# notu97/GS-SLAM-Analytica_Jacobian

Measured on AMD Instinct MI355X. Metric: Gaussian-pixel interactions/sec (fwd+Jacobian), 640x480, higher is better.
Workload: dtype f32; 1 GPU; cfg2: 50000 Gaussians (SH degree 3, 16 coeffs), 640x480; one step = one mapping window of 8 keyframes with distinct cameras: forward splat + analytical-Jacobian backward (dL/dmu, dL/dSigma->conic, per-Gaussian grads summed over the window, one dL/dtau per keyframe)

## Files before the change

gs-slam-analytica_jacobian_amd/csrc/preprocess.hip:

```cpp
#include "gsaj_common.h"
#include "wave_reduce.h"

__constant__ float kSH_C0 = 0.28209479177387814f;
__constant__ float kSH_C1 = 0.4886025119029199f;
__constant__ float kSH_C2[5] = {1.0925484305920792f, -1.0925484305920792f, 0.31539156525252005f, -1.0925484305920792f,
                                0.5462742152960396f};
__constant__ float kSH_C3[7] = {-0.5900435899266435f, 2.890611442640554f, -0.4570457994644658f, 0.3731763325901154f,
                                -0.4570457994644658f, 1.445305721320277f, -0.5900435899266435f};

__device__ __forceinline__ float3 ld3(const float *p, size_t i) { return make_float3(p[3 * i], p[3 * i + 1], p[3 * i + 2]); }

__device__ __forceinline__ void cov3d_from_scale_rot(float3 sc, float mod, float4 q, float *c6) {
  const float r = q.x, x = q.y, y = q.z, z = q.w;
  float R[3][3] = {{1.f - 2.f * (y * y + z * z), 2.f * (x * y - r * z), 2.f * (x * z + r * y)},
                   {2.f * (x * y + r * z), 1.f - 2.f * (x * x + z * z), 2.f * (y * z - r * x)},
                   {2.f * (x * z - r * y), 2.f * (y * z + r * x), 1.f - 2.f * (x * x + y * y)}};
  const float s[3] = {mod * sc.x, mod * sc.y, mod * sc.z};
  float A[3][3];
#pragma unroll
  for (int i = 0; i < 3; i++)
#pragma unroll
    for (int j = 0; j < 3; j++) A[i][j] = s[i] * R[j][i];
  float S[3][3];
#pragma unroll
  for (int a = 0; a < 3; a++)
#pragma unroll
    for (int b = a; b < 3; b++) S[a][b] = A[0][a] * A[0][b] + A[1][a] * A[1][b] + A[2][a] * A[2][b];
  c6[0] = S[0][0]; c6[1] = S[0][1]; c6[2] = S[0][2]; c6[3] = S[1][1]; c6[4] = S[1][2]; c6[5] = S[2][2];
}

__device__ __forceinline__ float3 cov2d_forward(float3 mean, float fx, float fy, float tanx, float tany, const float *c6,
                                                const float *vm) {
  float3 t = xform4x3(vm, mean);
  const float limx = 1.3f * tanx, limy = 1.3f * tany;
  const float txtz = t.x / t.z, tytz = t.y / t.z;
  t.x = fminf(limx, fmaxf(-limx, txtz)) * t.z;
  t.y = fminf(limy, fmaxf(-limy, tytz)) * t.z;
  const float J00 = fx / t.z, J02 = -(fx * t.x) / (t.z * t.z);
  const float J11 = fy / t.z, J12 = -(fy * t.y) / (t.z * t.z);
  float M[2][3];
#pragma unroll
  for (int k = 0; k < 3; k++) {
    M[0][k] = vm[4 * k + 0] * J00 + vm[4 * k + 1] * 0.0f + vm[4 * k + 2] * J02;
    M[1][k] = vm[4 * k + 0] * 0.0f + vm[4 * k + 1] * J11 + vm[4 * k + 2] * J12;
  }
  const float V[3][3] = {{c6[0], c6[1], c6[2]}, {c6[1], c6[3], c6[4]}, {c6[2], c6[4], c6[5]}};
  float X[2][3];
#pragma unroll
  for (int r = 0; r < 2; r++)
#pragma unroll
    for (int c = 0; c < 3; c++) X[r][c] = M[r][0] * V[c][0] + M[r][1] * V[c][1] + M[r][2] * V[c][2];
  float3 cov;
  cov.x = (X[0][0] * M[0][0] + X[0][1] * M[0][1] + X[0][2] * M[0][2]) + 0.3f;
  cov.y = X[1][0] * M[0][0] + X[1][1] * M[0][1] + X[1][2] * M[0][2];
  cov.z = (X[1][0] * M[1][0] + X[1][1] * M[1][1] + X[1][2] * M[1][2]) + 0.3f;
  return cov;
}

__device__ __forceinline__ float3 sh_to_rgb(int deg, float3 pos, float3 campos, const float *sh, uint8_t *clamped) {
  float3 d = make_float3(pos.x - campos.x, pos.y - campos.y, pos.z - campos.z);
  const float len = sqrtf(d.x * d.x + d.y * d.y + d.z * d.z);
  const float x = d.x / len, y = d.y / len, z = d.z / len;
  float out[3];
#pragma unroll
  for (int ch = 0; ch < 3; ch++) {
#define SHC(k) sh[(k) * 3 + ch]
    float res = kSH_C0 * SHC(0);
    if (deg > 0) {
      res = res - kSH_C1 * y * SHC(1) + kSH_C1 * z * SHC(2) - kSH_C1 * x * SHC(3);
      if (deg > 1) {
        const float xx = x * x, yy = y * y, zz = z * z, xy = x * y, yz = y * z, xz = x * z;
        res = res + kSH_C2[0] * xy * SHC(4) + kSH_C2[1] * yz * SHC(5) + kSH_C2[2] * (2.0f * zz - xx - yy) * SHC(6) +
              kSH_C2[3] * xz * SHC(7) + kSH_C2[4] * (xx - yy) * SHC(8);
        if (deg > 2) {
          res = res + kSH_C3[0] * y * (3.0f * xx - yy) * SHC(9) + kSH_C3[1] * xy * z * SHC(10) +
                kSH_C3[2] * y * (4.0f * zz - xx - yy) * SHC(11) + kSH_C3[3] * z * (2.0f * zz - 3.0f * xx - 3.0f * yy) * SHC(12) +
                kSH_C3[4] * x * (4.0f * zz - xx - yy) * SHC(13) + kSH_C3[5] * z * (xx - yy) * SHC(14) +
                kSH_C3[6] * x * (xx - 3.0f * yy) * SHC(15);
        }
      }
    }
#undef SHC
    res += 0.5f;
    clamped[ch] = (res < 0.0f);
    out[ch] = res < 0.0f ? 0.0f : res;
  }
  return make_float3(out[0], out[1], out[2]);
}

GSAJ_TRACE_DEFINE(pre)

template <bool SH16, bool MULTI>
__global__ __launch_bounds__(PRE_BLOCK) void k_preprocess(FwdParams p, int *__restrict__ radii, int *__restrict__ n_touched,
                                                         GeomWS g, ImageWS im, ViewStrides vs) {
  __shared__ uint32_t scan[PRE_BLOCK / 64];
  extern __shared__ uint32_t hist[];
  {
    const size_t view = blockIdx.y;
    g = geom_view(g, view * vs.geom);
    im = image_view(im, view * vs.image);
    p.viewmatrix += 16 * view;
    p.projmatrix += 16 * view;
    if (p.campos) p.campos += 3 * view;
    radii += view * (size_t)p.P;
    n_touched += view * (size_t)p.P;
  }
  GSAJ_TRACE_BEGIN(pre)
#ifdef GSAJ_BLOCK_TRACE
  unsigned long long trp_[4] = {0, 0, 0, 0}, trp_t = wall_clock64();
#define TRP(i) { const unsigned long long n_ = wall_clock64(); trp_[i] += n_ - trp_t; trp_t = n_; }
#else
#define TRP(i)
#endif
  const int tid = threadIdx.x;
  const int tiles = p.grid_x * p.grid_y;
  const bool use_lds = tiles <= LDS_TILES_MAX;
  if (use_lds) {
    for (int t = tid; t < tiles; t += PRE_BLOCK) hist[t] = 0u;
    __syncthreads();
  }
  const int nblk_all = (p.P + PRE_BLOCK - 1) / PRE_BLOCK;
#pragma clang loop unroll(disable)
  for (int it = 0; it < (MULTI ? p.bpw : 1); it++) {
  const int blk = MULTI ? (int)blockIdx.x * p.bpw + it : (int)blockIdx.x;
  if (blk >= nblk_all) break;
  const int idx = blk * PRE_BLOCK + tid;
  uint32_t touched = 0;
  uint32_t rect_x = 0, rect_y = 0;
  float depth = 0.f;
  if (idx < p.P) {
    int my_radius_i = 0;
    uint32_t rect_pack = 0;
    float2 xy = make_float2(0.f, 0.f);
    float4 con_o = make_float4(0.f, 0.f, 0.f, 0.f);
    float3 rgb = make_float3(0.f, 0.f, 0.f);
    uint8_t cl[3] = {0, 0, 0};
    float c6s[6] = {0.f, 0.f, 0.f, 0.f, 0.f, 0.f};
    const float3 p_orig = ld3(p.means3D, idx);
    float3 sc_in = make_float3(0.f, 0.f, 0.f);
    float4 q_in = make_float4(1.f, 0.f, 0.f, 0.f);
    if (!p.cov3D_precomp) {
      sc_in = ld3(p.scales, idx);
      q_in = reinterpret_cast<const float4 *>(p.rotations)[idx];
    }
    const float opac_in = p.opacities[idx];
    constexpr bool sh_regs = SH16;
    float shv[SH16 ? 48 : 1];
    if (sh_regs) {
      const float4 *s4 = reinterpret_cast<const float4 *>(p.shs + (size_t)idx * 48);
#pragma unroll
      for (int k = 0; k < 12; k++) {
        const float4 t = s4[k];
        shv[4 * k] = t.x; shv[4 * k + 1] = t.y; shv[4 * k + 2] = t.z; shv[4 * k + 3] = t.w;
      }
    }
    const float3 p_view = xform4x3(p.viewmatrix, p_orig);
    if (p_view.z <= 0.2f) {
      if (p.prefiltered) atomicOr(&im.counters[1], ERR_PREFILTERED);
    } else {
      const float4 p_hom = xform4x4(p.projmatrix, p_orig);
      const float p_w = 1.0f / (p_hom.w + 0.0000001f);
      const float3 p_proj = make_float3(p_hom.x * p_w, p_hom.y * p_w, p_hom.z * p_w);
      float c6[6];
      if (p.cov3D_precomp) {
#pragma unroll
        for (int k = 0; k < 6; k++) c6[k] = p.cov3D_precomp[6 * (size_t)idx + k];
      } else {
        cov3d_from_scale_rot(sc_in, p.scale_modifier, q_in, c6s);
#pragma unroll
        for (int k = 0; k < 6; k++) c6[k] = c6s[k];
      }
      const float3 cov = cov2d_forward(p_orig, p.focal_x, p.focal_y, p.tanfovx, p.tanfovy, c6, p.viewmatrix);
      const float det = cov.x * cov.z - cov.y * cov.y;
      if (det != 0.0f) {
        const float det_inv = 1.f / det;
        const float3 conic = make_float3(cov.z * det_inv, -cov.y * det_inv, cov.x * det_inv);
        const float mid = 0.5f * (cov.x + cov.z);
        const float sq = sqrtf(fmaxf(0.1f, mid * mid - det));
        const float lambda1 = mid + sq, lambda2 = mid - sq;
        const float my_radius = ceilf(3.f * sqrtf(fmaxf(lambda1, lambda2)));
        const float2 pim = make_float2(ndc2pix(p_proj.x, p.W), ndc2pix(p_proj.y, p.H));
        int x0, y0, x1, y1;
        tile_rect(pim.x, pim.y, (int)my_radius, p.grid_x, p.grid_y, gsaj_tile_band(im.sticky), x0, y0, x1, y1);
        const int area = (x1 - x0) * (y1 - y0);
        if (area != 0) {
          if (!p.colors_precomp) {
            const float3 cam = make_float3(p.campos[0], p.campos[1], p.campos[2]);
            if constexpr (sh_regs) rgb = sh_to_rgb(p.D, p_orig, cam, shv, cl);
            else rgb = sh_to_rgb(p.D, p_orig, cam, p.shs + (size_t)idx * p.M * 3, cl);
          }
          rect_pack = (uint32_t)x0 | ((uint32_t)y0 << 10) | ((uint32_t)(x1 - x0) << 20);
          rect_x = (uint32_t)x0 | ((uint32_t)x1 << 16);
          rect_y = (uint32_t)y0 | ((uint32_t)y1 << 16);
          depth = p_view.z;
          my_radius_i = (int)my_radius;
          xy = pim;
          con_o = make_float4(conic.x, conic.y, conic.z, opac_in);
          touched = (uint32_t)area;
          for (int y = y0; y < y1; y++)
            for (int x = x0; x < x1; x++) {
              if (use_lds) atomicAdd(&hist[y * p.grid_x + x], 1u);
              else atomicAdd(&im.tile_count[y * p.grid_x + x], 1u);
            }
        }
      }
    }
    radii[idx] = my_radius_i;
    n_touched[idx] = 0;
    g.depths[idx] = depth;
    if (!p.cov3D_precomp && blockIdx.y == 0) {
#pragma unroll
      for (int k = 0; k < 6; k++) g.cov3D[6 * (size_t)idx + k] = c6s[k];
    }
    if (!p.colors_precomp) {
      g.clamped[3 * (size_t)idx] = cl[0]; g.clamped[3 * (size_t)idx + 1] = cl[1]; g.clamped[3 * (size_t)idx + 2] = cl[2];
    }
    g.tiles_touched[idx] = touched;
    if (p.colors_precomp) rgb = ld3(p.colors_precomp, idx);
    g.splat[3 * (size_t)idx + 0] = make_float4(xy.x, xy.y, __uint_as_float(rect_pack), 0.f);
    g.splat[3 * (size_t)idx + 1] = con_o;
    g.splat[3 * (size_t)idx + 2] = make_float4(rgb.x, rgb.y, rgb.z, depth);
  }
  TRP(0)
  uint32_t incl = touched;
  {
    const int lane = tid & 63;
#pragma unroll
    for (int o = 1; o < 64; o <<= 1) {
      const uint32_t v = (uint32_t)__shfl_up((int)incl, o);
      if (lane >= o) incl += v;
    }
    if (lane == 63) scan[tid >> 6] = incl;
  }
  __syncthreads();
  uint32_t block_total = 0;
#pragma unroll
  for (int w = 0; w < PRE_BLOCK / 64; w++) {
    const uint32_t v = scan[w];
    if (w < (tid >> 6)) incl += v;
    block_total += v;
  }
  if (idx < p.P) {
    const uint32_t first = incl - touched;
    g.point_offsets[idx] = incl;
    reinterpret_cast<float *>(g.splat)[12 * (size_t)idx + 3] = __uint_as_float(first);
    g.scat[idx] = make_uint2(rect_x, rect_y);
  }
  if (tid == 0) g.block_sums[blk] = block_total;
  __syncthreads();
  }
  if (use_lds)
    for (int t = tid; t < tiles; t += PRE_BLOCK) {
      const uint32_t c = hist[t];
      if (c) atomicAdd(&im.tile_count[t], c);
    }
  TRP(1)
  GSAJ_TRACE_END(pre)
#ifdef GSAJ_BLOCK_TRACE
  if ((threadIdx.x & 63) == 0) {
    unsigned long long *t = g_trace_pre + 4 * (blockIdx.x * (PRE_BLOCK / 64) + (threadIdx.x >> 6));
    t[2] = (trp_[0] << 32) | trp_[1];
    t[3] = 0;
  }
#endif
}

__device__ uint32_t tail_exclusive_scan(const uint32_t *in, uint32_t *out, int n, uint32_t *run_max) {
  __shared__ uint32_t wsum[PRE_BLOCK / 64];
  __shared__ uint32_t wmax[PRE_BLOCK / 64];
  const int tid = threadIdx.x, lane = tid & 63, wave = tid >> 6;
  const int per = (n + PRE_BLOCK - 1) / PRE_BLOCK;
  const int b0 = min(n, tid * per), b1 = min(n, b0 + per);
  uint32_t s = 0, mx = 0;
  for (int i = b0; i < b1; i++) {
    const uint32_t v = in[i];
    s += v;
    mx = max(mx, v);
  }
  uint32_t incl = s;
#pragma unroll
  for (int o = 1; o < 64; o <<= 1) {
    const uint32_t v = __shfl_up((int)incl, o);
    if (lane >= o) incl += v;
  }
#pragma unroll
  for (int o = 32; o > 0; o >>= 1) mx = max(mx, (uint32_t)__shfl_xor((int)mx, o));
  if (lane == 63) wsum[wave] = incl;
  if (lane == 0) wmax[wave] = mx;
  __syncthreads();
  uint32_t woff = 0, total = 0, m = 0;
#pragma unroll
  for (int w = 0; w < PRE_BLOCK / 64; w++) {
    const uint32_t v = wsum[w];
    if (w < wave) woff += v;
    total += v;
    m = max(m, wmax[w]);
  }
  if (run_max) *run_max = m;
  uint32_t run = woff + incl - s;
  for (int i = b0; i < b1; i++) {
    const uint32_t v = in[i];
    out[i] = run;
    run += v;
  }
  __syncthreads();
  return total;
}

__device__ uint32_t tile_scan_and_schedule(int tiles, ImageWS im, uint32_t *len, uint32_t *longest_out) {
  __shared__ uint32_t wsum[PRE_BLOCK / 64], wmax[PRE_BLOCK / 64], cls[64];
  const int tid = threadIdx.x, lane = tid & 63, wave = tid >> 6;
  for (int c = tid; 4 * c < tiles; c += PRE_BLOCK) {
    const uint4 v = *reinterpret_cast<const uint4 *>(im.tile_count + 4 * c);
    len[4 * c] = v.x;
    if (4 * c + 1 < tiles) len[4 * c + 1] = v.y;
    if (4 * c + 2 < tiles) len[4 * c + 2] = v.z;
    if (4 * c + 3 < tiles) len[4 * c + 3] = v.w;
  }
  if (tid < 64) cls[tid] = 0u;
  __syncthreads();
  const int per = (tiles + PRE_BLOCK - 1) / PRE_BLOCK;
  const int b0 = min(tiles, tid * per), b1 = min(tiles, b0 + per);
  uint32_t s = 0, mx = 0;
  for (int i = b0; i < b1; i++) {
    s += len[i];
    mx = max(mx, len[i]);
  }
  uint32_t incl = s;
#pragma unroll
  for (int o = 1; o < 64; o <<= 1) {
    const uint32_t v = __shfl_up((int)incl, o);
    if (lane >= o) incl += v;
  }
#pragma unroll
  for (int o = 32; o > 0; o >>= 1) mx = max(mx, (uint32_t)__shfl_xor((int)mx, o));
  if (lane == 63) wsum[wave] = incl;
  if (lane == 0) wmax[wave] = mx;
  __syncthreads();
  uint32_t woff = 0, total = 0, longest = 0;
#pragma unroll
  for (int w = 0; w < PRE_BLOCK / 64; w++) {
    const uint32_t v = wsum[w];
    if (w < wave) woff += v;
    total += v;
    longest = max(longest, wmax[w]);
  }
  uint32_t run = woff + incl - s;
  for (int i = b0; i < b1; i++) {
    im.tile_offset[i] = run;
    run += len[i];
  }
  const int shift = longest >= 64u ? (32 - __builtin_clz(longest)) - 6 : 0;
  for (int t = tid; t < tiles; t += PRE_BLOCK) atomicAdd(&cls[63u - min(63u, len[t] >> shift)], 1u);
  __syncthreads();
  if (tid < 64) {
    const uint32_t v = cls[tid];
    uint32_t in2 = v;
#pragma unroll
    for (int o = 1; o < 64; o <<= 1) {
      const uint32_t u = (uint32_t)__shfl_up((int)in2, o);
      if (tid >= o) in2 += u;
    }
    cls[tid] = in2 - v;
  }
  __syncthreads();
  for (int t = tid; t < tiles; t += PRE_BLOCK) im.tile_order[atomicAdd(&cls[63u - min(63u, len[t] >> shift)], 1u)] = (uint32_t)t;
  __syncthreads();
  *longest_out = longest;
  return total;
}

__global__ __launch_bounds__(PRE_BLOCK) void k_frame_scan(int nblk, int tiles, int capacity, GeomWS g, ImageWS im, ViewStrides vs) {
  extern __shared__ uint32_t lds_len[];
  g = geom_view(g, (size_t)blockIdx.y * vs.geom);
  im = image_view(im, (size_t)blockIdx.y * vs.image);
  uint32_t *block_sums = g.block_sums;
  const uint32_t R = tail_exclusive_scan(block_sums, block_sums, nblk, nullptr);
  uint32_t m = 0, R2;
  if (tiles <= LDS_TILES_MAX) {
    R2 = tile_scan_and_schedule(tiles, im, lds_len, &m);
  } else {
    R2 = tail_exclusive_scan(im.tile_count, im.tile_offset, tiles, &m);
    for (int t = threadIdx.x; t < tiles; t += PRE_BLOCK) im.tile_order[t] = (uint32_t)t;
  }
  if (threadIdx.x == 0) {
    im.tile_offset[tiles] = R2;
    im.counters[0] = R;
    im.counters[2] = m;
    uint32_t err = 0u;
    if (R2 != R) err |= ERR_INTERNAL;
    if (capacity > 0) {
      if (R > (uint32_t)capacity) err |= ERR_CAPACITY;
      if (err) {
        im.counters[4] = 1u;
        atomicAdd(&im.sticky[0], 1u);
      }
    }
    if (err) atomicOr(&im.counters[1], err);
  }
}

#ifndef SCAT_CLS
#define SCAT_CLS 8
#endif
#define SCAT_LDS_TILES 4096
#define SCAT_STAGE 4096
GSAJ_TRACE_DEFINE(scat)

__global__ __launch_bounds__(PRE_BLOCK) void k_scatter_instances(int P, int gx, int gy, int gpt, GeomWS g, ImageWS im,
                                                                 uint32_t *__restrict__ inst_id, ViewStrides vs) {
  extern __shared__ uint32_t lds[];
  __shared__ uint32_t stage_id[SCAT_STAGE];
  __shared__ uint16_t stage_lt[SCAT_STAGE];
  __shared__ uint32_t s_wave[PRE_BLOCK / 64], s_carry;
  {
    const size_t view = blockIdx.y;
    g = geom_view(g, view * vs.geom);
    im = image_view(im, view * vs.image);
    inst_id = gsaj_shift(inst_id, view * vs.bin);
  }
  if (im.counters[4]) return;
  GSAJ_TRACE_BEGIN(scat)
#ifdef GSAJ_BLOCK_TRACE
  unsigned long long trs_[4] = {0, 0, 0, 0}, trs_t = wall_clock64();
#define TRS(i) { const unsigned long long n_ = wall_clock64(); trs_[i] += n_ - trs_t; trs_t = n_; }
#else
#define TRS(i)
#endif
  const int tid = threadIdx.x;
  const int cls = (int)(blockIdx.x % SCAT_CLS), gb = (int)(blockIdx.x / SCAT_CLS);
  const int rows_c = (gy - cls + SCAT_CLS - 1) / SCAT_CLS;
  const int ltiles = rows_c > 0 ? rows_c * gx : 0;
  const bool use_lds = ((gy + SCAT_CLS - 1) / SCAT_CLS) * gx <= SCAT_LDS_TILES;
  uint32_t *cnt = lds, *fill = lds + ltiles, *lbase = lds + 2 * ltiles;
  if (use_lds) {
    for (int t = tid; t < 2 * ltiles; t += PRE_BLOCK) lds[t] = 0u;
    if (tid == 0) s_carry = 0u;
    __syncthreads();
  }
#define SCAT_FOR_EACH_TILE(BODY)                                                                     \
  for (int i0 = 0; i0 < gpt; i0 += 4) {                                                              \
    uint2 sc[4];                                                                                     \
    _Pragma("unroll") for (int j = 0; j < 4; j++) {                                                  \
      const int idx = (gb * gpt + i0 + j) * PRE_BLOCK + tid;                                         \
      sc[j] = (i0 + j < gpt && idx < P) ? g.scat[idx] : make_uint2(0u, 0u);                          \
    }                                                                                                \
    _Pragma("unroll") for (int j = 0; j < 4; j++) {                                                  \
      const int x0 = (int)(sc[j].x & 0xffffu), x1 = (int)(sc[j].x >> 16);                            \
      const int y0 = (int)(sc[j].y & 0xffffu), y1 = (int)(sc[j].y >> 16);                            \
      if (x1 > x0) {                                                                                 \
        const uint32_t id = (uint32_t)((gb * gpt + i0 + j) * PRE_BLOCK + tid);                       \
        (void)id;                                                                                    \
        const int ys = y0 + ((cls - y0) % SCAT_CLS + SCAT_CLS) % SCAT_CLS;                           \
        for (int y = ys; y < y1; y += SCAT_CLS)                                                      \
          for (int x = x0; x < x1; x++) {                                                            \
            const int lt = (y / SCAT_CLS) * gx + x;                            \
            const int t = y * gx + x;                                                      \
            (void)lt; (void)t;                                                                       \
            BODY                                                                                     \
          }                                                                                          \
      }                                                                                              \
    }                                                                                                \
  }
  if (!use_lds) {
    SCAT_FOR_EACH_TILE({ inst_id[im.tile_offset[t] + atomicAdd(&im.tile_cursor[t], 1u)] = id; })
    return;
  }
  TRS(0)
  SCAT_FOR_EACH_TILE({ atomicAdd(&cnt[lt], 1u); })
  __syncthreads();
  TRS(1)
  for (int l0 = 0; l0 < ltiles; l0 += PRE_BLOCK) {
    const int lt = l0 + tid, lane = tid & 63;
    uint32_t c = 0u, off = 0u, base = 0u;
    if (lt < ltiles) {
      const int j = lt / gx;
      const int t = (j * SCAT_CLS + cls) * gx + (lt - j * gx);
      c = cnt[lt];
      off = im.tile_offset[t];
      if (c) base = atomicAdd(&im.tile_cursor[t], c);
    }
    uint32_t incl = c;
#pragma unroll
    for (int o = 1; o < 64; o <<= 1) {
      const uint32_t v = (uint32_t)__shfl_up((int)incl, o);
      if (lane >= o) incl += v;
    }
    if (lane == 63) s_wave[tid >> 6] = incl;
    __syncthreads();
    uint32_t before = s_carry;
#pragma unroll
    for (int w = 0; w < PRE_BLOCK / 64; w++)
      if (w < (tid >> 6)) before += s_wave[w];
    if (lt < ltiles) {
      cnt[lt] = off + base;
      lbase[lt] = before + incl - c;
    }
    __syncthreads();
    if (tid == PRE_BLOCK - 1) s_carry = before + incl;
  }
  __syncthreads();
  const uint32_t total = s_carry;
  TRS(2)
  if (total <= SCAT_STAGE) {
    SCAT_FOR_EACH_TILE({
      const uint32_t k = atomicAdd(&fill[lt], 1u);
      stage_id[lbase[lt] + k] = id;
      stage_lt[lbase[lt] + k] = (uint16_t)lt;
    })
    __syncthreads();
    for (uint32_t i = tid; i < total; i += PRE_BLOCK) {
      const uint32_t lt = stage_lt[i];
      inst_id[cnt[lt] + (i - lbase[lt])] = stage_id[i];
    }
  } else {
    SCAT_FOR_EACH_TILE({ inst_id[cnt[lt] + atomicAdd(&fill[lt], 1u)] = id; })
  }
#undef SCAT_FOR_EACH_TILE
  TRS(3)
  GSAJ_TRACE_END(scat)
#ifdef GSAJ_BLOCK_TRACE
  if ((threadIdx.x & 63) == 0) {
    const unsigned tw_ = (blockIdx.y * gridDim.x + blockIdx.x) * (blockDim.x >> 6) + (threadIdx.x >> 6);
    if (tw_ < GSAJ_TRACE_MAX) {
      g_trace_scat[4 * tw_ + 2] = (trs_[0] << 32) | trs_[1];
      g_trace_scat[4 * tw_ + 3] = (trs_[2] << 32) | trs_[3];
    }
  }
#endif
}

__global__ __launch_bounds__(256) void k_pack_splat16(int P, GeomWS g, const uint32_t *__restrict__ counters, ViewStrides vs) {
  g = geom_view(g, (size_t)blockIdx.y * vs.geom);
  if (gsaj_shift(counters, (size_t)blockIdx.y * vs.image)[4]) return;
  const int idx = blockIdx.x * 256 + threadIdx.x;
  if (idx >= P) return;
  const float4 a = g.splat[3 * (size_t)idx + 0], bq = g.splat[3 * (size_t)idx + 1], c = g.splat[3 * (size_t)idx + 2];
  g.splat16[2 * (size_t)idx + 0] = make_float4(a.x, a.y, c.w, a.w);
  g.splat16[2 * (size_t)idx + 1] = make_float4(__uint_as_float(gsaj_pack_h2(bq.x, bq.y)), __uint_as_float(gsaj_pack_h2(bq.z, bq.w)),
                                              __uint_as_float(gsaj_pack_h2(c.x, c.y)), __uint_as_float(gsaj_pack_h2(c.z, 0.f)));
}

template <int J>
__device__ __forceinline__ uint32_t lane_xor(uint32_t x, int lane) {
  if (J == 32) {
    const gsaj_u32x2 r = __builtin_amdgcn_permlane32_swap(x, x, false, false);
    return lane < 32 ? r[1] : r[0];
  } else if (J == 16) {
    const gsaj_u32x2 r = __builtin_amdgcn_permlane16_swap(x, x, false, false);
    return (lane & 16) ? r[0] : r[1];
  } else if (J == 8) {
    return (uint32_t)__builtin_amdgcn_mov_dpp((int)x, 0x128, 0xF, 0xF, true);
  } else if (J == 4) {
    int t = __builtin_amdgcn_mov_dpp((int)x, 0x104, 0xF, 0x5, false);
    t = __builtin_amdgcn_update_dpp(t, (int)x, 0x114, 0xF, 0xA, false);
    return (uint32_t)t;
  } else if (J == 2) {
    return (uint32_t)__builtin_amdgcn_mov_dpp((int)x, 0x4E, 0xF, 0xF, true);
  } else {
    return (uint32_t)__builtin_amdgcn_mov_dpp((int)x, 0xB1, 0xF, 0xF, true);
  }
}
template <int MASK>
__device__ __forceinline__ uint32_t lane_mirror(uint32_t x, int lane) {
  if (MASK == 1) return (uint32_t)__builtin_amdgcn_mov_dpp((int)x, 0xB1, 0xF, 0xF, true);
  else if (MASK == 3) return (uint32_t)__builtin_amdgcn_mov_dpp((int)x, 0x1B, 0xF, 0xF, true);
  else if (MASK == 7) return (uint32_t)__builtin_amdgcn_mov_dpp((int)x, 0x141, 0xF, 0xF, true);
  else if (MASK == 15) return (uint32_t)__builtin_amdgcn_mov_dpp((int)x, 0x140, 0xF, 0xF, true);
  else if (MASK == 31) return lane_xor<16>(lane_mirror<15>(x, lane), lane);
  else return lane_xor<32>(lane_mirror<31>(x, lane), lane);
}
template <int MASK>
__device__ __forceinline__ uint64_t key_mirror(uint64_t k, int lane) {
  return ((uint64_t)lane_mirror<MASK>((uint32_t)(k >> 32), lane) << 32) | lane_mirror<MASK>((uint32_t)k, lane);
}

#define KEY_INF 0x7FEFFFFFFFFFFFFFull
__device__ __forceinline__ void key_minmax(uint64_t a, uint64_t b, uint64_t &lo, uint64_t &hi) {
  double l, h;
  asm("v_min_f64 %0, %2, %3\n\tv_max_f64 %1, %2, %3" : "=&v"(l), "=&v"(h) : "v"(__longlong_as_double((long long)a)), "v"(__longlong_as_double((long long)b)));
  lo = (uint64_t)__double_as_longlong(l);
  hi = (uint64_t)__double_as_longlong(h);
}
__device__ __forceinline__ uint64_t key_min(uint64_t a, uint64_t b) {
  double l;
  asm("v_min_f64 %0, %1, %2" : "=v"(l) : "v"(__longlong_as_double((long long)a)), "v"(__longlong_as_double((long long)b)));
  return (uint64_t)__double_as_longlong(l);
}
__device__ __forceinline__ uint64_t key_max(uint64_t a, uint64_t b) {
  double h;
  asm("v_max_f64 %0, %1, %2" : "=v"(h) : "v"(__longlong_as_double((long long)a)), "v"(__longlong_as_double((long long)b)));
  return (uint64_t)__double_as_longlong(h);
}
template <int J>
__device__ __forceinline__ constexpr uint64_t lower_lanes() {
  return J == 1 ? 0x5555555555555555ull : J == 2 ? 0x3333333333333333ull : J == 4 ? 0x0F0F0F0F0F0F0F0Full
       : J == 8 ? 0x00FF00FF00FF00FFull : J == 16 ? 0x0000FFFF0000FFFFull : 0x00000000FFFFFFFFull;
}
__device__ __forceinline__ void key_stage(uint64_t &A, uint64_t XA, uint64_t YA, uint64_t &B, uint64_t XB, uint64_t YB, uint64_t lower) {
  double a, b2;
  uint64_t save;
  asm volatile("s_mov_b64 %[sv], exec\n\t"
               "s_and_b64 exec, %[sv], %[lo]\n\t"
               "v_min_f64 %[a], %[xa], %[ya]\n\t"
               "v_min_f64 %[b], %[xb], %[yb]\n\t"
               "s_andn2_b64 exec, %[sv], %[lo]\n\t"
               "v_max_f64 %[a], %[xa], %[ya]\n\t"
               "v_max_f64 %[b], %[xb], %[yb]\n\t"
               "s_mov_b64 exec, %[sv]\n\t"
               "s_nop 4"
               : [a] "=&v"(a), [b] "=&v"(b2), [sv] "=&s"(save)
               : [xa] "v"(__longlong_as_double((long long)XA)), [ya] "v"(__longlong_as_double((long long)YA)),
                 [xb] "v"(__longlong_as_double((long long)XB)), [yb] "v"(__longlong_as_double((long long)YB)), [lo] "s"(lower)
               : "scc");
  A = (uint64_t)__double_as_longlong(a);
  B = (uint64_t)__double_as_longlong(b2);
}
template <int J>
__device__ __forceinline__ void key_both(uint64_t k, uint64_t &of_lower, uint64_t &of_upper) {
  const uint32_t hi = (uint32_t)(k >> 32), lo = (uint32_t)k;
  gsaj_u32x2 rh, rl;
  if (J == 32) {
    rh = __builtin_amdgcn_permlane32_swap(hi, hi, false, false);
    rl = __builtin_amdgcn_permlane32_swap(lo, lo, false, false);
    of_lower = ((uint64_t)rh[0] << 32) | rl[0];
    of_upper = ((uint64_t)rh[1] << 32) | rl[1];
  } else {
    rh = __builtin_amdgcn_permlane16_swap(hi, hi, false, false);
    rl = __builtin_amdgcn_permlane16_swap(lo, lo, false, false);
    of_lower = ((uint64_t)rh[0] << 32) | rl[0];
    of_upper = ((uint64_t)rh[1] << 32) | rl[1];
  }
}
template <int J>
__device__ __forceinline__ void sort_stage(uint64_t &A, uint64_t &B, int lane) {
  if constexpr (J >= 16) {
    uint64_t al, au, bl, bu;
    key_both<J>(A, al, au);
    key_both<J>(B, bl, bu);
    key_stage(A, al, au, B, bl, bu, lower_lanes<J>());
  } else {
    const uint64_t PA = ((uint64_t)lane_xor<J>((uint32_t)(A >> 32), lane) << 32) | lane_xor<J>((uint32_t)A, lane);
    const uint64_t PB = ((uint64_t)lane_xor<J>((uint32_t)(B >> 32), lane) << 32) | lane_xor<J>((uint32_t)B, lane);
    key_stage(A, A, PA, B, B, PB, lower_lanes<J>());
  }
}
template <int J>
__device__ __forceinline__ void merge_strides(uint64_t &A, uint64_t &B, int lane) {
  if constexpr (J == 64) {
    key_minmax(A, B, A, B);
  } else {
    sort_stage<J>(A, B, lane);
  }
  if constexpr (J > 1) merge_strides<J / 2>(A, B, lane);
}
template <int K>
__device__ __forceinline__ void local_merge(uint64_t &A, uint64_t &B, int lane) {
  if constexpr (K == 128) {
    const uint64_t PA = key_mirror<63>(B, lane), PB = key_mirror<63>(A, lane);
    A = key_min(A, PA);
    B = key_max(B, PB);
    merge_strides<32>(A, B, lane);
  } else {
    const uint64_t PA = key_mirror<K - 1>(A, lane), PB = key_mirror<K - 1>(B, lane);
    key_stage(A, A, PA, B, B, PB, lower_lanes<K / 2>());
    if constexpr (K >= 4) merge_strides<K / 4>(A, B, lane);
  }
}
template <int K>
__device__ __forceinline__ void local_merges(uint64_t &A, uint64_t &B, int lane, int m) {
  if (K > m) return;
  local_merge<K>(A, B, lane);
  if constexpr (K < 128) local_merges<2 * K>(A, B, lane, m);
}

template <int NT>
__device__ __forceinline__ void lds_bitonic_sort(uint64_t *keys, int n, int tid) {
  const int lane = tid & 63, wave = tid >> 6;
  const int nch = (n + 127) >> 7, nup = nch << 7;
  int m = 2;
  while (m < n) m <<= 1;
  for (int chunk = wave; chunk < nch; chunk += NT / 64) {
    const int ia = chunk * 128 + lane, ib = ia + 64;
    uint64_t A = keys[ia], B = keys[ib];
    local_merges<2>(A, B, lane, m);
    keys[ia] = A;
    keys[ib] = B;
  }
  __syncthreads();
  for (int k = 256, hs = 7; (k >> 1) < nup; k <<= 1, hs++) {
    const int half = k >> 1;
    for (int i = tid; i < (nup >> 1) + half; i += NT) {
      const int blk = i >> hs, off = i & (half - 1);
      const int l = (blk << (hs + 1)) + off, r = (blk << (hs + 1)) + k - 1 - off;
      if (r < nup) key_minmax(keys[l], keys[r], keys[l], keys[r]);
    }
    __syncthreads();
    for (int j = k >> 2; j >= 128; j >>= 1) {
      for (int i = tid; i < (nup >> 1); i += NT) {
        const int l = ((i & ~(j - 1)) << 1) | (i & (j - 1)), r = l + j;
        if (r < nup && ((l & ~(k - 1)) + half) < nup) key_minmax(keys[l], keys[r], keys[l], keys[r]);
      }
      __syncthreads();
    }
    for (int chunk = wave; chunk < nch; chunk += NT / 64) {
      if (((chunk * 128) & ~(k - 1)) + half >= nup) continue;
      const int ia = chunk * 128 + lane, ib = ia + 64;
      uint64_t A = keys[ia], B = keys[ib];
      merge_strides<64>(A, B, lane);
      keys[ia] = A;
      keys[ib] = B;
    }
    __syncthreads();
  }
}

template <int NT>
__device__ __forceinline__ void lds_bitonic_merge(uint64_t *keys, int T, int tid) {
  const int lane = tid & 63, wave = tid >> 6;
  for (int j = T >> 1; j >= 128; j >>= 1) {
    for (int i = tid; i < (T >> 1); i += NT) {
      const int l = ((i & ~(j - 1)) << 1) | (i & (j - 1)), r = l + j;
      key_minmax(keys[l], keys[r], keys[l], keys[r]);
    }
    __syncthreads();
  }
  for (int chunk = wave; chunk * 128 < T; chunk += NT / 64) {
    const int ia = chunk * 128 + lane, ib = ia + 64;
    uint64_t A = keys[ia], B = keys[ib];
    merge_strides<64>(A, B, lane);
    keys[ia] = A;
    keys[ib] = B;
  }
  __syncthreads();
}

template <int NT>
__device__ const uint64_t *sort_long_list(uint64_t *lds, int T, uint32_t *split_s, const uint32_t *ids, const float *__restrict__ depths,
                                          uint64_t *a, uint64_t *b, int n, int tid) {
  for (int c0 = 0; c0 < n; c0 += T) {
    const int len = min(T, n - c0);
    for (int i0 = tid; i0 < T; i0 += 4 * NT) {
      uint32_t id[4], dz[4];
#pragma unroll
      for (int u = 0; u < 4; u++) id[u] = ids[c0 + min(i0 + u * NT, len - 1)];
#pragma unroll
      for (int u = 0; u < 4; u++) dz[u] = __float_as_uint(depths[id[u]]);
#pragma unroll
      for (int u = 0; u < 4; u++) asm volatile("" : "+v"(dz[u]));
#pragma unroll
      for (int u = 0; u < 4; u++) {
        const int i = i0 + u * NT;
        if (i < T) lds[i] = i < len ? ((uint64_t)dz[u] << 32) | id[u] : KEY_INF;
      }
    }
    __syncthreads();
    lds_bitonic_sort<NT>(lds, T, tid);
    for (int i = tid; i < len; i += NT) b[c0 + i] = lds[i];
    __syncthreads();
  }
  uint64_t *src = b, *dst = a;
  for (long long width = T; width < (long long)n; width <<= 1) {
    asm volatile("s_waitcnt vmcnt(0)" ::: "memory");
    __syncthreads();
    for (long long p0 = 0; p0 < (long long)n; p0 += 2 * width) {
      const int la = (int)min(width, (long long)n - p0);
      const int lb = (int)max(0ll, min(width, (long long)n - p0 - width));
      const uint64_t *A = src + p0, *B = src + p0 + width;
      uint64_t *D = dst + p0;
      if (lb == 0) {
        for (int i = tid; i < la; i += NT) D[i] = A[i];
        continue;
      }
      const int tot = la + lb, nblk = (tot + T - 1) / T;
      for (int j0 = 0; j0 < nblk; j0 += PRE_BLOCK) {
        for (int t = tid; t <= PRE_BLOCK; t += NT) {
          const long long dl = (long long)(j0 + t) * T;
          const int d = (int)min(dl, (long long)tot);
          int lo = max(0, d - lb), hi = min(d, la);
          while (lo < hi) {
            const int mid = (lo + hi) >> 1;
            if (A[mid] <= B[d - 1 - mid]) lo = mid + 1;
            else hi = mid;
          }
          split_s[t] = (uint32_t)lo;
        }
        __syncthreads();
        for (int j = j0; j < min(nblk, j0 + PRE_BLOCK); j++) {
          const int a0 = (int)split_s[j - j0], a1 = (int)split_s[j - j0 + 1];
          const int d0 = j * T, d1 = min(tot, d0 + T);
          const int b0 = d0 - a0, cA = a1 - a0, cB = (d1 - a1) - b0;
          for (int i = tid; i < T; i += NT) lds[i] = i < cA ? A[a0 + i] : (i >= T - cB ? B[b0 + (T - 1 - i)] : KEY_INF);
          __syncthreads();
          lds_bitonic_merge<NT>(lds, T, tid);
          for (int i = tid; i < cA + cB; i += NT) D[d0 + i] = lds[i];
          __syncthreads();
        }
      }
    }
    uint64_t *t = src;
    src = dst;
    dst = t;
  }
  asm volatile("s_waitcnt vmcnt(0)" ::: "memory");
  __syncthreads();
  return src;
}

GSAJ_TRACE_DEFINE(sort)

#ifndef GSAJ_SORT_128_MAX
#define GSAJ_SORT_128_MAX 1024
#endif
template <int NT>
__global__ __launch_bounds__(NT) void k_tile_sort(ImageWS im, const float *__restrict__ depths, uint64_t *__restrict__ inst_key,
                                                   uint64_t *__restrict__ keys_b, uint32_t *point_list,
                                                   uint8_t *__restrict__ reached, int cap, int pass, int rec16, ViewStrides vs) {
  {
    const size_t view = blockIdx.y;
    im = image_view(im, view * vs.image);
    depths = gsaj_shift(depths, view * vs.geom);
    inst_key = gsaj_shift(inst_key, view * vs.bin);
    keys_b = gsaj_shift(keys_b, view * vs.bin);
    point_list = gsaj_shift(point_list, view * vs.bin);
    reached = gsaj_shift(reached, view * vs.bin);
  }
  extern __shared__ uint64_t keys[];
  if (im.counters[4]) return;
  GSAJ_TRACE_BEGIN(sort)
#ifdef GSAJ_BLOCK_TRACE
  unsigned long long tr_a = wall_clock64(), tr_b = 0, tr_c = 0;
#endif
  const int tid = threadIdx.x, tile = blockIdx.x;
  const uint32_t beg = im.tile_offset[tile * TILE_REP], end = im.tile_offset[(tile + 1) * TILE_REP];
  const int n = (int)(end - beg);
  if (pass != 2) {
    if (tid == 0) im.ranges[tile] = n > 0 ? make_uint2(beg, end) : make_uint2(0u, 0u);
    if (tid == 0 && tile == 0) im.counters[7] = (uint32_t)rec16;
    for (uint32_t k = beg + tid; k < end; k += NT) reached[k] = 0;
  }
  if (n == 0) return;
  const uint64_t *sorted = keys;
  if (n > cap) {
    if (pass == 2) return;
    const int T = cap >= 4096 ? cap / 2 : cap;
    sorted = sort_long_list<NT>(keys, T, reinterpret_cast<uint32_t *>(keys + T), point_list + beg, depths, inst_key + beg, keys_b + beg, n, tid);
  } else {
    int m = 2;
    while (m < n) m <<= 1;
    if (pass == 1 && 2 * m <= cap) return;
    if (pass == 2 && m > cap) return;
    const int nup = ((n + 127) >> 7) << 7;
    for (int i0 = tid; i0 < nup; i0 += 4 * NT) {
      uint32_t id[4], dz[4];
#pragma unroll
      for (int u = 0; u < 4; u++) id[u] = point_list[beg + (uint32_t)min(i0 + u * NT, n - 1)];
#pragma unroll
      for (int u = 0; u < 4; u++) dz[u] = __float_as_uint(depths[id[u]]);
#pragma unroll
      for (int u = 0; u < 4; u++) asm volatile("" : "+v"(dz[u]));
#pragma unroll
      for (int u = 0; u < 4; u++) {
        const int i = i0 + u * NT;
        if (i < nup) keys[i] = i < n ? ((uint64_t)dz[u] << 32) | id[u] : KEY_INF;
      }
    }
    __syncthreads();
#ifdef GSAJ_BLOCK_TRACE
    tr_b = wall_clock64();
#endif
    lds_bitonic_sort<NT>(keys, n, tid);
  }
#ifdef GSAJ_BLOCK_TRACE
  tr_c = wall_clock64();
#endif
  for (int i = tid; i < n; i += NT) point_list[beg + (uint32_t)i] = (uint32_t)sorted[i];
  GSAJ_TRACE_END(sort)
#ifdef GSAJ_BLOCK_TRACE
  if ((threadIdx.x & 63) == 0) {
    unsigned long long *t = g_trace_sort + 4 * (blockIdx.x * (NT / 64) + (threadIdx.x >> 6));
    t[2] = tr_b - tr_a;
    t[3] = tr_c - tr_b;
  }
#endif
}

__global__ __launch_bounds__(PRE_BLOCK) void k_mark_visible(int P, const float *__restrict__ means3D,
                                                            const float *__restrict__ vm, uint8_t *__restrict__ present) {
  const int idx = blockIdx.x * PRE_BLOCK + threadIdx.x;
  if (idx >= P) return;
  const float3 pv = xform4x3(vm, ld3(means3D, idx));
  present[idx] = pv.z > 0.2f;
}

__global__ __launch_bounds__(256) void k_zero_frame_state(uint32_t *__restrict__ counters, size_t words, size_t view_stride) {
  uint32_t *c = gsaj_shift(counters, blockIdx.y * view_stride);
  for (size_t i = (size_t)blockIdx.x * 256 + threadIdx.x; i < words; i += (size_t)gridDim.x * 256) c[i] = 0u;
}

int launch_preprocess(const FwdParams &p0, int *radii, int *n_touched, const GeomWS &g, const ImageWS &im, ViewStrides vs,
                      hipStream_t s) {
  FwdParams p = p0;
  const int nblk = (p.P + PRE_BLOCK - 1) / PRE_BLOCK;
  const int views = p.views > 0 ? p.views : 1;
  p.bpw = 1;
  while (p.bpw < 8 && (long long)nblk * views / (2 * p.bpw) >= 4096) p.bpw *= 2;
  const int nwg = (nblk + p.bpw - 1) / p.bpw;
  {
    const size_t words = im.zero_bytes / sizeof(uint32_t);
    hipLaunchKernelGGL(k_zero_frame_state, dim3((unsigned)((words + 1023) / 1024), views), dim3(256), 0, s, im.counters, words,
                       vs.image);
  }
  {
    GsajProfScope ps(ST_PREPROCESS, s);
    const int tiles = p.grid_x * p.grid_y;
    const size_t lds = tiles <= LDS_TILES_MAX ? sizeof(uint32_t) * (size_t)tiles : 0;
#ifndef GSAJ_PRE_NO_SHREGS
    if (!p.colors_precomp && p.M == 16)
#else
    if (false)
#endif
      if (p.bpw > 1) hipLaunchKernelGGL((k_preprocess<true, true>), dim3(nwg, views), dim3(PRE_BLOCK), lds, s, p, radii, n_touched, g, im, vs);
      else hipLaunchKernelGGL((k_preprocess<true, false>), dim3(nwg, views), dim3(PRE_BLOCK), lds, s, p, radii, n_touched, g, im, vs);
    else
      if (p.bpw > 1) hipLaunchKernelGGL((k_preprocess<false, true>), dim3(nwg, views), dim3(PRE_BLOCK), lds, s, p, radii, n_touched, g, im, vs);
      else hipLaunchKernelGGL((k_preprocess<false, false>), dim3(nwg, views), dim3(PRE_BLOCK), lds, s, p, radii, n_touched, g, im, vs);
    hipLaunchKernelGGL(k_frame_scan, dim3(1, views), dim3(PRE_BLOCK), lds, s, nblk, tiles, p.capacity, g, im, vs);
  }
  GSAJ_HIP_CHECK(hipGetLastError());
  return GSAJ_OK;
}

int launch_tile_binning(int P, int sort_cap, int rec16, int grid_x, int grid_y, const GeomWS &g, const BinWS &b, const ImageWS &im,
                        int views, ViewStrides vs, hipStream_t s) {
  {
    GsajProfScope ps(ST_SCATTER, s);
    const int ltiles = ((grid_y + SCAT_CLS - 1) / SCAT_CLS) * grid_x;
    const size_t lds = ltiles <= SCAT_LDS_TILES ? 3 * sizeof(uint32_t) * (size_t)ltiles : 0;
    int gpt = 4;
    while (gpt < 8 && (long long)P * views * SCAT_CLS / ((long long)PRE_BLOCK * gpt * 2) >= 1536) gpt *= 2;
    for (int g2 = 9; gpt == 8 && g2 <= 10; g2++) {
      const long long wg8 = (long long)((P + PRE_BLOCK * 8 - 1) / (PRE_BLOCK * 8)) * SCAT_CLS * views;
      const long long wg2 = (long long)((P + PRE_BLOCK * g2 - 1) / (PRE_BLOCK * g2)) * SCAT_CLS * views;
      if (wg8 > 1536 && wg2 <= 1536) gpt = g2;
    }
    const int per = PRE_BLOCK * gpt;
    hipLaunchKernelGGL(k_scatter_instances, dim3((unsigned)((P + per - 1) / per) * SCAT_CLS, views), dim3(PRE_BLOCK), lds, s, P, grid_x,
                       grid_y, gpt, g, im, b.point_list, vs);
    if (rec16)
      hipLaunchKernelGGL(k_pack_splat16, dim3((P + 255) / 256, views), dim3(256), 0, s, P, g, im.counters, vs);
  }
  {
    GsajProfScope ps(ST_TILE_SORT, s);
    int cap = 128;
    while (cap < sort_cap && cap < SORT_CAP) cap <<= 1;
    if (sizeof(uint64_t) * (size_t)cap > 65536)
      (void)hipFuncSetAttribute(reinterpret_cast<const void *>(&k_tile_sort<512>), hipFuncAttributeMaxDynamicSharedMemorySize,
                                (int)(sizeof(uint64_t) * (size_t)cap));
    const size_t split_bytes = cap >= 4096 ? 0 : sizeof(uint32_t) * (PRE_BLOCK + 1);
    auto launch = [&](int lds_keys, int pass, size_t extra) {
      const size_t dyn = sizeof(uint64_t) * (size_t)lds_keys + extra;
      if (lds_keys >= 4096)
        hipLaunchKernelGGL(k_tile_sort<512>, dim3(grid_x * grid_y, views), dim3(512), dyn, s, im, g.depths, b.keys_unsorted, b.keys,
                           b.point_list, b.reached, lds_keys, pass, rec16, vs);
      else if (lds_keys > GSAJ_SORT_128_MAX)
        hipLaunchKernelGGL(k_tile_sort<256>, dim3(grid_x * grid_y, views), dim3(256), dyn, s, im, g.depths, b.keys_unsorted, b.keys,
                           b.point_list, b.reached, lds_keys, pass, rec16, vs);
      else
        hipLaunchKernelGGL(k_tile_sort<128>, dim3(grid_x * grid_y, views), dim3(128), dyn, s, im, g.depths, b.keys_unsorted, b.keys,
                           b.point_list, b.reached, lds_keys, pass, rec16, vs);
    };
    if (cap >= 4096) {
      launch(cap, 1, 0);
      launch(cap / 2, 2, 0);
    } else {
      launch(cap, 0, split_bytes);
    }
  }
  GSAJ_HIP_CHECK(hipGetLastError());
  return GSAJ_OK;
}

int launch_mark_visible(int P, const float *means3D, const float *viewmatrix, uint8_t *present, hipStream_t s) {
  const int nblk = (P + PRE_BLOCK - 1) / PRE_BLOCK;
  hipLaunchKernelGGL(k_mark_visible, dim3(nblk), dim3(PRE_BLOCK), 0, s, P, means3D, viewmatrix, present);
  GSAJ_HIP_CHECK(hipGetLastError());
  return GSAJ_OK;
}
```

Baseline: 735.4 billion interactions/s.

## Sort several tiles per workgroup with prefetch of next tile's keys

Adds a persistent-style tile sort kernel in which each workgroup sorts up to eight tiles in turn. While the current tile is being sorted in LDS, it prefetches the next tile's ids and depths and defers the point_list write-back. The goal is to hide global load latency and cut launch and workgroup overhead when there are more tiles than resident workgroups. The tiles-per-workgroup count comes from the CU count and can be overridden with an environment variable. The costs are higher register pressure from holding the prefetched data and lower parallelism when tiles are uneven.

Measured after the change: 723.8 billion interactions/s. 1.6% lower.

```diff
diff --git a/gs-slam-analytica_jacobian_amd/csrc/preprocess.hip b/gs-slam-analytica_jacobian_amd/csrc/preprocess.hip
--- a/gs-slam-analytica_jacobian_amd/csrc/preprocess.hip
+++ b/gs-slam-analytica_jacobian_amd/csrc/preprocess.hip
@@ -1,3 +1,5 @@
+#include <stdlib.h>
+
 #include "gsaj_common.h"
 #include "wave_reduce.h"
 
@@ -675,9 +677,9 @@
 }
 
 template <int NT>
-__device__ __forceinline__ void lds_bitonic_sort(uint64_t *keys, int n, int tid) {
+__device__ __forceinline__ void lds_sort_chunks(uint64_t *keys, int n, int tid) {
   const int lane = tid & 63, wave = tid >> 6;
-  const int nch = (n + 127) >> 7, nup = nch << 7;
+  const int nch = (n + 127) >> 7;
   int m = 2;
   while (m < n) m <<= 1;
   for (int chunk = wave; chunk < nch; chunk += NT / 64) {
@@ -687,6 +689,11 @@
     keys[ia] = A;
     keys[ib] = B;
   }
+}
+template <int NT>
+__device__ __forceinline__ void lds_sort_merges(uint64_t *keys, int n, int tid) {
+  const int lane = tid & 63, wave = tid >> 6;
+  const int nch = (n + 127) >> 7, nup = nch << 7;
   __syncthreads();
   for (int k = 256, hs = 7; (k >> 1) < nup; k <<= 1, hs++) {
     const int half = k >> 1;
@@ -714,6 +721,11 @@
     __syncthreads();
   }
 }
+template <int NT>
+__device__ __forceinline__ void lds_bitonic_sort(uint64_t *keys, int n, int tid) {
+  lds_sort_chunks<NT>(keys, n, tid);
+  lds_sort_merges<NT>(keys, n, tid);
+}
 
 template <int NT>
 __device__ __forceinline__ void lds_bitonic_merge(uint64_t *keys, int T, int tid) {
@@ -736,7 +748,7 @@
 }
 
 template <int NT>
-__device__ const uint64_t *sort_long_list(uint64_t *lds, int T, uint32_t *split_s, const uint32_t *ids, const float *__restrict__ depths,
+__device__ __forceinline__ const uint64_t *sort_long_list(uint64_t *lds, int T, uint32_t *split_s, const uint32_t *ids, const float *__restrict__ depths,
                                           uint64_t *a, uint64_t *b, int n, int tid) {
   for (int c0 = 0; c0 < n; c0 += T) {
     const int len = min(T, n - c0);
@@ -885,6 +897,145 @@
 #endif
 }
 
+#define SORT_TILES_MAX 8
+template <int NT, int RPT>
+__global__ __launch_bounds__(NT, 8) __attribute__((amdgpu_num_sgpr(80))) void k_tile_sort_multi(
+    ImageWS im, const float *__restrict__ depths, uint64_t *__restrict__ inst_key, uint64_t *__restrict__ keys_b, uint32_t *point_list,
+    uint8_t *__restrict__ reached, int cap, int tiles, int rec16, ViewStrides vs) {
+  static_assert(RPT % 4 == 0, "entries are requested four at a time");
+  {
+    const size_t view = blockIdx.y;
+    im = image_view(im, view * vs.image);
+    depths = gsaj_shift(depths, view * vs.geom);
+    inst_key = gsaj_shift(inst_key, view * vs.bin);
+    keys_b = gsaj_shift(keys_b, view * vs.bin);
+    point_list = gsaj_shift(point_list, view * vs.bin);
+    reached = gsaj_shift(reached, view * vs.bin);
+  }
+  extern __shared__ uint64_t keys[];
+  __shared__ uint32_t sched[SORT_TILES_MAX][4];
+  if (im.counters[4] || (int)blockIdx.x >= tiles) return;
+  GSAJ_TRACE_BEGIN(sort)
+#ifdef GSAJ_BLOCK_TRACE
+  unsigned long long tr_load = 0, tr_sort = 0;
+#endif
+  const int tid = threadIdx.x, G = (int)gridDim.x;
+  const int wbase = __builtin_amdgcn_readfirstlane(tid & ~63);
+  const int cnt = min((tiles - 1 - (int)blockIdx.x) / G + 1, SORT_TILES_MAX);
+  if (tid < cnt) {
+    const int t = (int)min(im.tile_order[blockIdx.x + tid * G], (uint32_t)(tiles - 1));
+    sched[tid][0] = (uint32_t)t;
+    sched[tid][1] = im.tile_offset[t * TILE_REP];
+    sched[tid][2] = im.tile_offset[(t + 1) * TILE_REP];
+  }
+  if (tid == 0 && blockIdx.x == 0) im.counters[7] = (uint32_t)rec16;
+  __syncthreads();
+  uint32_t id[RPT], dz[RPT];
+  uint32_t out[RPT];
+  bool have = false, pend = false;
+  uint32_t pbeg = 0;
+  int pn = 0;
+  auto flush = [&]() {
+#pragma unroll
+    for (int u = 0; u < RPT; u++)
+      if (tid + u * NT < pn) point_list[pbeg + (uint32_t)(tid + u * NT)] = out[u];
+    pend = false;
+  };
+  for (int it = 0; it < cnt; it++) {
+#ifdef GSAJ_BLOCK_TRACE
+    const unsigned long long tr_a = wall_clock64();
+#endif
+    const int tile = __builtin_amdgcn_readfirstlane((int)sched[it][0]);
+    const uint32_t beg = (uint32_t)__builtin_amdgcn_readfirstlane((int)sched[it][1]);
+    const uint32_t end = (uint32_t)__builtin_amdgcn_readfirstlane((int)sched[it][2]);
+    const int n = (int)(end - beg);
+    if (n == 0 || n > cap) {
+      if (pend) flush();
+      if (tid == 0) im.ranges[tile] = n > 0 ? make_uint2(beg, end) : make_uint2(0u, 0u);
+      if (n == 0) continue;
+      for (uint32_t k = beg + tid; k < end; k += NT) reached[k] = 0;
+      const int T = cap;
+      const uint64_t *sorted =
+          sort_long_list<NT>(keys, T, reinterpret_cast<uint32_t *>(keys + T), point_list + beg, depths, inst_key + beg, keys_b + beg, n, tid);
+      for (int i = tid; i < n; i += NT) point_list[beg + (uint32_t)i] = (uint32_t)sorted[i];
+      continue;
+    }
+    const int nup = ((n + 127) >> 7) << 7;
+    if (!have) {
+#pragma unroll
+      for (int g = 0; g < RPT; g += 4) {
+        if (wbase + g * NT < nup) {
+#pragma unroll
+          for (int u = g; u < g + 4; u++) id[u] = point_list[beg + (uint32_t)min(tid + u * NT, n - 1)];
+#pragma unroll
+          for (int u = g; u < g + 4; u++) dz[u] = __float_as_uint(depths[id[u]]);
+#pragma unroll
+          for (int u = g; u < g + 4; u++) asm volatile("" : "+v"(dz[u]));
+        }
+      }
+    }
+#pragma unroll
+    for (int u = 0; u < RPT; u++) {
+      const int i = tid + u * NT;
+      if (i < nup) keys[i] = i < n ? ((uint64_t)dz[u] << 32) | id[u] : KEY_INF;
+    }
+    __syncthreads();
+#ifdef GSAJ_BLOCK_TRACE
+    const unsigned long long tr_b = wall_clock64();
+#endif
+    if (pend) flush();
+    if (tid == 0) im.ranges[tile] = make_uint2(beg, end);
+    for (uint32_t k = beg + tid; k < end; k += NT) reached[k] = 0;
+    uint32_t nbeg = 0;
+    int nn = 0;
+    if (it + 1 < cnt) {
+      nbeg = (uint32_t)__builtin_amdgcn_readfirstlane((int)sched[it + 1][1]);
+      nn = (int)((uint32_t)__builtin_amdgcn_readfirstlane((int)sched[it + 1][2]) - nbeg);
+    }
+    const bool pre = nn > 0 && nn <= cap;
+    const int nnup = ((nn + 127) >> 7) << 7;
+    if (pre) {
+#pragma unroll
+      for (int g = 0; g < RPT; g += 4)
+        if (wbase + g * NT < nnup) {
+#pragma unroll
+          for (int u = g; u < g + 4; u++) id[u] = point_list[nbeg + (uint32_t)min(tid + u * NT, nn - 1)];
+        }
+    }
+    lds_sort_chunks<NT>(keys, n, tid);
+    if (pre) {
+#pragma unroll
+      for (int g = 0; g < RPT; g += 4)
+        if (wbase + g * NT < nnup) {
+#pragma unroll
+          for (int u = g; u < g + 4; u++) dz[u] = __float_as_uint(depths[id[u]]);
+        }
+    }
+    lds_sort_merges<NT>(keys, n, tid);
+#ifdef GSAJ_BLOCK_TRACE
+    tr_load += tr_b - tr_a;
+    tr_sort += wall_clock64() - tr_b;
+#endif
+#pragma unroll
+    for (int u = 0; u < RPT; u++)
+      if (tid + u * NT < n) out[u] = (uint32_t)keys[tid + u * NT];
+    pbeg = beg;
+    pn = n;
+    pend = true;
+    have = pre;
+    if (it + 1 < cnt) __syncthreads();
+  }
+  if (pend) flush();
+  GSAJ_TRACE_END(sort)
+#ifdef GSAJ_BLOCK_TRACE
+  if ((threadIdx.x & 63) == 0) {
+    unsigned long long *t = g_trace_sort + 4 * (blockIdx.x * (NT / 64) + (threadIdx.x >> 6));
+    t[2] = tr_load;
+    t[3] = tr_sort;
+  }
+#endif
+}
+
 __global__ __launch_bounds__(PRE_BLOCK) void k_mark_visible(int P, const float *__restrict__ means3D,
                                                             const float *__restrict__ vm, uint8_t *__restrict__ present) {
   const int idx = blockIdx.x * PRE_BLOCK + threadIdx.x;
@@ -928,6 +1079,21 @@
     hipLaunchKernelGGL(k_frame_scan, dim3(1, views), dim3(PRE_BLOCK), lds, s, nblk, tiles, p.capacity, g, im, vs);
   }
   GSAJ_HIP_CHECK(hipGetLastError());
+  return GSAJ_OK;
+}
+
+static int sort_resident_workgroups(int nt, int *out) {
+  static int cus[64];
+  int dev = 0;
+  GSAJ_HIP_CHECK(hipGetDevice(&dev));
+  const int slot = dev >= 0 && dev < 64 ? dev : 0;
+  int n = cus[slot];
+  if (n <= 0) {
+    GSAJ_HIP_CHECK(hipDeviceGetAttribute(&n, hipDeviceAttributeMultiprocessorCount, dev));
+    if (n <= 0) n = 1;
+    if (dev == slot) cus[slot] = n;
+  }
+  *out = n * (32 / (nt / 64));
   return GSAJ_OK;
 }
 
@@ -974,7 +1140,29 @@
       launch(cap, 1, 0);
       launch(cap / 2, 2, 0);
     } else {
-      launch(cap, 0, split_bytes);
+      const int tiles = grid_x * grid_y, nt = cap > GSAJ_SORT_128_MAX ? 256 : 128;
+      int resident = 0, per = 1;
+      if (int rc = sort_resident_workgroups(nt, &resident)) return rc;
+      while (per < SORT_TILES_MAX && (long long)views * ((tiles + per - 1) / per) > resident) per++;
+      if (const char *e = getenv("GSAJ_SORT_TILES_PER_WG")) {
+        const int forced = atoi(e);
+        if (forced >= 1) per = forced < SORT_TILES_MAX ? forced : SORT_TILES_MAX;
+      }
+      if (per == 1) {
+        launch(cap, 0, split_bytes);
+      } else {
+        const dim3 grid((tiles + per - 1) / per, views);
+        const size_t dyn = sizeof(uint64_t) * (size_t)cap + split_bytes;
+        if (nt == 256)
+          hipLaunchKernelGGL((k_tile_sort_multi<256, 8>), grid, dim3(256), dyn, s, im, g.depths, b.keys_unsorted, b.keys, b.point_list,
+                             b.reached, cap, tiles, rec16, vs);
+        else if (cap > 512)
+          hipLaunchKernelGGL((k_tile_sort_multi<128, 8>), grid, dim3(128), dyn, s, im, g.depths, b.keys_unsorted, b.keys, b.point_list,
+                             b.reached, cap, tiles, rec16, vs);
+        else
+          hipLaunchKernelGGL((k_tile_sort_multi<128, 4>), grid, dim3(128), dyn, s, im, g.depths, b.keys_unsorted, b.keys, b.point_list,
+                             b.reached, cap, tiles, rec16, vs);
+      }
     }
   }
   GSAJ_HIP_CHECK(hipGetLastError());
```
